# mpeg5/xeve

Measured on AMD Instinct MI355X. Metric: encoded frames/sec @ 2160p Baseline medium; SAD-kernel HBM GB/s vs peak, higher is better.
Workload: dtype s16 samples, s32/s64 accumulation, f64 cost comparisons (bit-exact)

## Files before the change

### xeve_amd/csrc/rdo.hip

```cpp
#include <cstdlib>
#include "xh_common.h"
#include "mc_cu.h"

extern "C" int xeve_hip_residual_rdoq_dev(const pel *org, int s_org, const pel *pred, int s_pred, const xeve_hip_job *jobs, int njobs, int log2w, int log2h,
                                          int bit_depth, int qp, int qscale, int dqscale, int is_intra_slice, double lambda, int ch_type, int tool_iqt,
                                          const xeve_hip_rdoq_est_full *est, const int32_t *est_idx, int16_t *coef, pel *rec, int s_rec, int32_t *nnz,
                                          int64_t *ssd, void *stream);

struct RdoK {
    int    n0, n1, ncomp, njobs, dir_unused;
    int    w, h, ws, hs, s_org_l, s_org_c;
    double lambda[3], wgt[2];
};

struct Cand {
    double cost_best;
    int    nnz_store[3], idx_best[3], cbf_idx[3], iy, iu, iv, tnnz, round4, win;
};

#define MAX_COST 1.7e+308

__device__ __forceinline__ void copy_state(xeve_hip_sbac *d, const xeve_hip_sbac *s)
{
    const unsigned *a = (const unsigned *)s;
// ... 208 lines not shown
}

__global__ void k_rdo_spec_decide(const xeve_hip_rdo_job *__restrict__ jobs, RdoK P, const long *ssd_y, const long *ssd_u, const long *ssd_v,
                                  const unsigned *__restrict__ bits, const unsigned *__restrict__ cbits, const xeve_hip_sbac *__restrict__ st_out,
                                  Cand *__restrict__ cand, xeve_hip_rdo_result *__restrict__ res, unsigned char *__restrict__ drop, xeve_hip_sbac *__restrict__ best)
{
    const int j = blockIdx.x * blockDim.x + threadIdx.x;
    if(j >= P.njobs) return;
    const xeve_hip_rdo_job J = jobs[j];
    Cand c = cand[j];
    long d0[3], d1[3];
    load_dist(ssd_y, ssd_u, ssd_v, j, P, d0, d1);
    const size_t N = P.njobs;
    auto wb = [&](int k) { return (double)(int)bits[(size_t)k * N + j]; };
    auto cb = [&](int lane, int which) { return (double)(int)cbits[4 * ((size_t)lane * N + j) + which]; };
    if(c.tnnz == 0) {
        c.cost_best = (double)d0[0] + (P.wgt[0] * (double)d0[1]) + (P.wgt[1] * (double)d0[2]);
        c.cost_best += wb(0) * P.lambda[0];
        c.win = 0;
        if(best) copy_state(best + j, st_out + j);
    }
    else {
        if(!J.dir_flag) {
            double cost = sum_cost(d0, d1, 0, 0, 0, P);
            cost += wb(0) * P.lambda[0];
            if(cost < c.cost_best) {
                c.cost_best = cost, c.cbf_idx[0] = c.cbf_idx[1] = c.cbf_idx[2] = 0, c.win = 0;
                if(best) copy_state(best + j, st_out + j);
            }
        }
        {
            double cost = sum_cost(d0, d1, c.iy, c.iu, c.iv, P);
            cost += wb(7) * P.lambda[0];
            if(cost < c.cost_best) {
                c.cost_best = cost, c.cbf_idx[0] = c.iy, c.cbf_idx[1] = c.iu, c.cbf_idx[2] = c.iv, c.win = 1;
                if(best) copy_state(best + j, st_out + 7 * N + j);
            }
        }
        int lane = 0;
        if(c.nnz_store[0] > 0) {
            double c0 = (double)d0[0] * 1.0, c1 = (double)d1[0] * 1.0;
            c0 += cb(0, 0) * P.lambda[0], c1 += cb(1, 0) * P.lambda[0];
            c.idx_best[0] = c1 < c0;
            lane |= c.idx_best[0];
        }
        if(c.nnz_store[1] > 0) {
            double c0 = (double)d0[1] * P.wgt[0], c1 = (double)d1[1] * P.wgt[0];
            c0 += cb(lane, 1) * P.lambda[1], c1 += cb(lane | 2, 1) * P.lambda[1];
            c.idx_best[1] = c1 < c0;
            lane |= c.idx_best[1] << 1;
        }
        if(c.nnz_store[2] > 0) {
            double c0 = (double)d0[2] * P.wgt[1], c1 = (double)d1[2] * P.wgt[1];
            c0 += cb(lane, 2) * P.lambda[2], c1 += cb(lane, 3) * P.lambda[2];
            c.idx_best[2] = c1 < c0;
        }
        int n[3] = {c.nnz_store[0], c.nnz_store[1], c.nnz_store[2]};
        if(c.idx_best[0] || c.idx_best[1] || c.idx_best[2]) {
            c.iy = c.idx_best[0], c.iu = c.idx_best[1], c.iv = c.idx_best[2];
            n[0] = c.iy ? n[0] : 0, n[1] = c.iu ? n[1] : 0, n[2] = c.iv ? n[2] : 0;
        }
        c.round4 = n[0] != c.nnz_store[0] || n[1] != c.nnz_store[1] || n[2] != c.nnz_store[2];
        if(c.round4) {
            const int k = (n[0] ? 1 : 0) | (n[1] ? 2 : 0) | (n[2] ? 4 : 0);
            double cost = sum_cost(d0, d1, c.iy, c.iu, c.iv, P);
            cost += wb(k) * P.lambda[0];
            if(cost < c.cost_best) {
                c.cost_best = cost, c.cbf_idx[0] = c.iy, c.cbf_idx[1] = c.iu, c.cbf_idx[2] = c.iv, c.win = 2;
                if(best) copy_state(best + j, st_out + (size_t)k * N + j);
            }
        }
    }
    cand[j] = c;
    xeve_hip_rdo_result r;
    r.cost = c.cost_best, r.pad_ = 0;
    for(int k = 0; k < 3; k++) {
        r.nnz[k] = c.tnnz != 0 && c.cbf_idx[k] ? c.nnz_store[k] : 0;
        drop[3 * j + k] = r.nnz[k] == 0 && c.nnz_store[k] != 0;
        r.dist[0][k] = d0[k], r.dist[1][k] = c.tnnz != 0 ? d1[k] : 0;
    }
    res[j] = r;
}

static int rdo_spec_limit()
{
    static const int v = getenv("XEVE_HIP_RDO_SPEC") ? atoi(getenv("XEVE_HIP_RDO_SPEC")) : 256;
    return v;
}
static bool rdo_use_spec(int njobs) { return njobs <= rdo_spec_limit(); }

static size_t al(size_t v) { return (v + 255) & ~(size_t)255; }

struct RdoLayout {
    size_t mc, rl, rc, est_idx, est, pred[3], rec[3], nnz[3], ssd[3], cand, prev, bj, bits, st_out, drop, mcws, bitws, total;
};
static RdoLayout rdo_layout(int njobs, int n0, int n1, int nstates, size_t rec_l, size_t rec_c, int w, int h, int nr0, int nr1)
{
    RdoLayout L;
    size_t o = 0, n = njobs;
    auto take = [&](size_t bytes) { size_t r = o; o += al(bytes); return r; };
    L.mc = take(n * sizeof(xeve_hip_cu_mc_job)), L.rl = take(n * sizeof(xeve_hip_job)), L.rc = take(n * sizeof(xeve_hip_job));
    L.est_idx = take(n * 4), L.est = take((size_t)nstates * sizeof(xeve_hip_rdoq_est_full));
    L.pred[0] = take(n * n0 * 2), L.pred[1] = take(n * n1 * 2 + 8), L.pred[2] = take(n * n1 * 2 + 8);
    (void)rec_l, (void)rec_c;
    L.rec[0] = take(n * n0 * 2), L.rec[1] = take(n * n1 * 2 + 8), L.rec[2] = take(n * n1 * 2 + 8);
    for(int k = 0; k < 3; k++) L.nnz[k] = take(n * 4), L.ssd[k] = take(n * 16);
    L.cand = take(n * sizeof(Cand)), L.prev = take(n * sizeof(xeve_hip_sbac));
    const size_t kinds = rdo_use_spec(njobs) ? 8 : 4;
    L.bj = take((kinds + 4) * n * sizeof(xeve_hip_cu_bits_job)), L.bits = take((kinds + 16) * n * 4), L.st_out = take(kinds * n * sizeof(xeve_hip_sbac));
    L.drop = take(3 * n);
    L.mcws = take(xeve_hip_mc_cu_workspace(njobs, w, h, nr0, nr1));
    L.bitws = take(xeve_hip_cu_bits_workspace((int)kinds * njobs, n * ((size_t)n0 + 2 * (size_t)n1)));
    L.total = o;
    return L;
}

extern "C" size_t xeve_hip_residue_rdo_workspace(int njobs, int nstates, const xeve_hip_rdo_params *p, int s_org_l, int s_org_c)
{
    if(!p || njobs <= 0) return 256;
    const int ws = p->chroma_format_idc <= 2, hs = p->chroma_format_idc <= 1;
    const int n0 = 1 << (p->log2_cuw + p->log2_cuh), n1 = p->chroma_format_idc ? n0 >> (ws + hs) : 0;
    return rdo_layout(njobs, n0, n1, nstates > 0 ? nstates : 1, (size_t)s_org_l * p->pic_h, (size_t)s_org_c * (p->pic_h >> hs), 1 << p->log2_cuw, 1 << p->log2_cuh,
                      p->num_refp[0], p->num_refp[1]).total;
}

static const int k_q_scale[6]  = {26214, 23302, 20560, 18396, 16384, 14764};
static const int k_dq_scale[6] = {40, 45, 51, 57, 64, 71};

extern "C" int xeve_hip_residue_rdo_jobs(const xeve_hip_pel *const org[3], int s_org_l, int s_org_c, const xeve_hip_refpic *refp, int s_l, int s_c,
                                         const xeve_hip_sbac *states, int nstates, const xeve_hip_rdo_params *p, const xeve_hip_rdo_job *jobs, int njobs,
                                         const int16_t (*coef_l)[8], const int16_t (*coef_c)[4], xeve_hip_rdo_result *results, int16_t *coef,
                                         xeve_hip_sbac *best, void *workspace, size_t workspace_bytes, void *stream)
{
    return xh_residue_rdo_jobs_x(org, s_org_l, s_org_c, refp, s_l, s_c, states, nstates, p, jobs, njobs, coef_l, coef_c, results, coef, best, workspace, workspace_bytes, stream,
                                 nullptr, 0);
}

int xh_residue_rdo_jobs_x(const xeve_hip_pel *const org[3], int s_org_l, int s_org_c, const xeve_hip_refpic *refp, int s_l, int s_c, const xeve_hip_sbac *states, int nstates,
                          const xeve_hip_rdo_params *p, const xeve_hip_rdo_job *jobs, int njobs, const int16_t (*coef_l)[8], const int16_t (*coef_c)[4],
                          xeve_hip_rdo_result *results, int16_t *coef, xeve_hip_sbac *best, void *workspace, size_t workspace_bytes, void *stream,
                          const void *est_shared, int keep_dropped)
{
    XH_ENTER();
    XH_REQUIRE(org && refp && states && nstates > 0 && p && jobs && njobs >= 0 && results && coef && workspace && coef_l);
    XH_REQUIRE(p->log2_cuw >= 2 && p->log2_cuw <= 6 && p->log2_cuh >= 2 && p->log2_cuh <= 6 && p->tool_iqt == 0);
    XH_REQUIRE(p->chroma_format_idc == 0 || p->chroma_format_idc == 1 || p->chroma_format_idc == 3);
    XH_REQUIRE(org[0] && (p->chroma_format_idc == 0 || (org[1] && org[2] && coef_c)));
    if(njobs == 0) return XEVE_HIP_OK;
    XH_REQUIRE(workspace_bytes >= xeve_hip_residue_rdo_workspace(njobs, nstates, p, s_org_l, s_org_c));
    const int idc = p->chroma_format_idc, ws = idc <= 2, hs = idc <= 1, bd = p->bit_depth;
    const int lw[3] = {p->log2_cuw, p->log2_cuw - ws, p->log2_cuw - ws}, lh[3] = {p->log2_cuh, p->log2_cuh - hs, p->log2_cuh - hs};
    RdoK P;
    P.n0 = 1 << (lw[0] + lh[0]), P.n1 = idc ? 1 << (lw[1] + lh[1]) : 0, P.ncomp = idc ? 3 : 1, P.njobs = njobs, P.dir_unused = 0;
    P.w = 1 << lw[0], P.h = 1 << lh[0], P.ws = ws, P.hs = hs, P.s_org_l = s_org_l, P.s_org_c = s_org_c;
    for(int k = 0; k < 3; k++) P.lambda[k] = p->lambda[k];
    P.wgt[0] = p->dist_chroma_weight[0], P.wgt[1] = p->dist_chroma_weight[1];
    const RdoLayout L = rdo_layout(njobs, P.n0, P.n1, nstates, (size_t)s_org_l * p->pic_h, (size_t)s_org_c * (p->pic_h >> hs), P.w, P.h, p->num_refp[0], p->num_refp[1]);
    char *W = (char *)workspace;
    auto *rl = (xeve_hip_job *)(W + L.rl), *rc = (xeve_hip_job *)(W + L.rc);
    int  *est_idx = (int *)(W + L.est_idx);
    auto *est = est_shared ? (xeve_hip_rdoq_est_full *)est_shared : (xeve_hip_rdoq_est_full *)(W + L.est);
    pel  *pred[3] = {(pel *)(W + L.pred[0]), (pel *)(W + L.pred[1]), (pel *)(W + L.pred[2])};
    pel  *rec[3]  = {(pel *)(W + L.rec[0]), (pel *)(W + L.rec[1]), (pel *)(W + L.rec[2])};
    int  *nnz[3]  = {(int *)(W + L.nnz[0]), (int *)(W + L.nnz[1]), (int *)(W + L.nnz[2])};
    long *ssd[3]  = {(long *)(W + L.ssd[0]), (long *)(W + L.ssd[1]), (long *)(W + L.ssd[2])};
    auto *cand = (Cand *)(W + L.cand);
    auto *prev = (xeve_hip_sbac *)(W + L.prev), *st_out = (xeve_hip_sbac *)(W + L.st_out);
    auto *bj = (xeve_hip_cu_bits_job *)(W + L.bj);
    auto *bits = (unsigned *)(W + L.bits);
    auto *drop = (unsigned char *)(W + L.drop);
    hipStream_t st = (hipStream_t)stream;
    const int   G  = (njobs + 255) / 256;
    int rc_;

    CuMcPrep C;
    rc_ = xh_mc_cu_prep_params(refp, p->num_refp[0], p->num_refp[1], p->pic_w, p->pic_h, njobs, P.w, P.h, idc, W + L.mcws, L.bitws - L.mcws, &C);
    if(rc_ != XEVE_HIP_OK) return rc_;
    k_rdo_prep<<<G, 256, 0, st>>>(jobs, P, C, rl, rc, est_idx);
    rc_ = xh_mc_cu_jobs_x(refp, p->num_refp[0], p->num_refp[1], s_l, s_c, p->pic_w, p->pic_h, nullptr, njobs, P.w, P.h, bd, bd, idc, coef_l, coef_c, pred[0],
                          pred[1], pred[2], W + L.mcws, L.bitws - L.mcws, stream, XH_MC_PREPPED);
    if(rc_ != XEVE_HIP_OK) return rc_;
    if(!est_shared) {
        rc_ = xeve_hip_rdoq_bit_est(states, nstates, est, stream);
        if(rc_ != XEVE_HIP_OK) return rc_;
    }
    int16_t *cf[3] = {coef, coef + (size_t)njobs * P.n0, coef + (size_t)njobs * (P.n0 + P.n1)};
    for(int k = 0; k < P.ncomp; k++) {
        const int q = p->qp[k];
        XH_REQUIRE(q >= 0 && q <= 51 + 6 * (bd - 8));
        rc_ = xeve_hip_residual_rdoq_dev(org[k], k ? s_org_c : s_org_l, pred[k], 1 << lw[k], k ? rc : rl, njobs, lw[k], lh[k], bd, q, k_q_scale[q % 6],
                                         k_dq_scale[q % 6] << (q / 6), p->slice_type == 2, p->lambda[k], k, p->tool_iqt, est, est_idx, cf[k], rec[k],
                                         -(1 << lw[k]), nnz[k], (int64_t *)ssd[k], stream);
        if(rc_ != XEVE_HIP_OK) return rc_;
    }
    xeve_hip_cu_bits_params bp;
    bp.log2_cuw = p->log2_cuw, bp.log2_cuh = p->log2_cuh, bp.slice_type = p->slice_type, bp.num_refp[0] = p->num_refp[0], bp.num_refp[1] = p->num_refp[1];
    bp.cm_init = 0, bp.chroma_format_idc = idc;
    const size_t coef_elems = (size_t)njobs * (P.n0 + 2 * (size_t)P.n1), bws = workspace_bytes - L.bitws;
    if(rdo_use_spec(njobs)) {
        xeve_hip_cu_bits_job *cj = bj + 8 * (size_t)njobs;
        unsigned             *cbits = bits + 8 * (size_t)njobs;
        k_rdo_spec_jobs<<<G, 256, 0, st>>>(jobs, P, nnz[0], nnz[1], nnz[2], cand, bj, cj);
        rc_ = xh_cu_bits_jobs_round(coef, coef_elems, states, bj, 8 * njobs, &bp, W + L.bitws, bws, bits, best ? st_out : nullptr, best != nullptr, 0, stream, 7 * njobs, njobs);
        if(rc_ != XEVE_HIP_OK) return rc_;
        rc_ = xh_cu_bits_chain_round(coef_elems, states, cj, 4 * njobs, &bp, W + L.bitws, bws, cbits, stream);
        if(rc_ != XEVE_HIP_OK) return rc_;
        k_rdo_spec_decide<<<G, 256, 0, st>>>(jobs, P, ssd[0], ssd[1], ssd[2], bits, cbits, st_out, cand, results, drop, best);
        if(!keep_dropped) k_rdo_zero_dropped<<<(3 * njobs + 3) / 4, 256, 0, st>>>(coef, drop, P);
        XH_HIP(hipGetLastError());
        return XEVE_HIP_OK;
    }
    k_rdo_round1<<<G, 256, 0, st>>>(jobs, P, nnz[0], nnz[1], nnz[2], cand, bj);
    rc_ = xh_cu_bits_jobs_round(coef, coef_elems, states, bj, 4 * njobs, &bp, W + L.bitws, bws, bits, st_out, best != nullptr, 0, stream, njobs, njobs);
    if(rc_ != XEVE_HIP_OK) return rc_;
    k_rdo_decide1<<<G, 256, 0, st>>>(jobs, P, ssd[0], ssd[1], ssd[2], bits, st_out, states, cand, prev, bj, best);
    if(P.ncomp > 1) {
        for(int comp = 1; comp <= 2; comp++) {
            rc_ = xh_cu_bits_jobs_round(coef, coef_elems, prev, bj, 2 * njobs, &bp, W + L.bitws, bws, bits, st_out, 0, 1, stream);
            if(rc_ != XEVE_HIP_OK) return rc_;
            k_rdo_decide_comp<<<G, 256, 0, st>>>(jobs, P, comp, ssd[0], ssd[1], ssd[2], bits, st_out, cand, prev, bj);
        }
    }
    else k_rdo_decide_comp<<<G, 256, 0, st>>>(jobs, P, 2, ssd[0], ssd[1], ssd[2], bits, st_out, cand, prev, bj);
    rc_ = xh_cu_bits_jobs_round(coef, coef_elems, states, bj, njobs, &bp, W + L.bitws, bws, bits, best ? st_out : nullptr, best != nullptr, 1, stream);
    if(rc_ != XEVE_HIP_OK) return rc_;
    k_rdo_finish<<<G, 256, 0, st>>>(jobs, P, ssd[0], ssd[1], ssd[2], bits, cand, results, drop, st_out, best);
    if(!keep_dropped) k_rdo_zero_dropped<<<(3 * njobs + 3) / 4, 256, 0, st>>>(coef, drop, P);
    XH_HIP(hipGetLastError());
    return XEVE_HIP_OK;
}

struct SkipK {
    int    njobs, S, mc, isb, n0, n1, ncomp, ws, hs, s_org_l, s_org_c, best_shift;
    double lambda0, wgt[2];
};

__global__ void k_skip_prep(const xeve_hip_skip_job *__restrict__ jobs, SkipK P, CuMcPrep C, xeve_hip_cu_mc_job *__restrict__ mc, xeve_hip_job *__restrict__ rl,
                            xeve_hip_job *__restrict__ rc, xeve_hip_cu_bits_job *__restrict__ bj, unsigned char *__restrict__ valid, int *__restrict__ zero)
{
    const int t = blockIdx.x * blockDim.x + threadIdx.x;
    if(t < 64) zero[t] = 0;
    if(t >= P.njobs * P.S) return;
    const int j = t / P.S, s = t % P.S;
    const int i0 = P.isb ? s / P.mc : s, i1 = P.isb ? s % P.mc : 0;
    const xeve_hip_skip_job J = jobs[j];
    const int cnt1 = P.isb ? J.ncand : 1;
    bool ok = i0 < J.ncand && i1 < cnt1;
    for(int k = 0; k < 3; k++) {
        if(k < i0 && J.mvp[0][k][0] == J.mvp[0][i0][0] && J.mvp[0][k][1] == J.mvp[0][i0][1]) ok = false;
        if(k < i1 && J.mvp[1][k][0] == J.mvp[1][i1][0] && J.mvp[1][k][1] == J.mvp[1][i1][1]) ok = false;
    }
    xeve_hip_cu_mc_job m;
    m.x = J.x, m.y = J.y, m.mv[0][0] = J.mvp[0][i0][0], m.mv[0][1] = J.mvp[0][i0][1], m.mv[1][0] = J.mvp[1][i1][0], m.mv[1][1] = J.mvp[1][i1][1];
    m.refi[0] = J.refi_pred[0][i0], m.refi[1] = P.isb ? J.refi_pred[1][i1] : -1, m.pad_[0] = m.pad_[1] = 0;
    if(m.refi[0] < 0 && m.refi[1] < 0) ok = false;
    if(!ok) m.refi[0] = m.refi[1] = -1;
    mc[t] = m;
    xh_cu_mc_prep_one(m, t, C);
    rl[t] = xh_make_job(J.y, P.s_org_l, J.x, t * P.n0);
    rc[t] = xh_make_job(J.y >> P.hs, P.s_org_c, J.x >> P.ws, t * P.n1);
    xeve_hip_cu_bits_job b;
    b.coef_off[0] = b.coef_off[1] = b.coef_off[2] = 0, b.nnz[0] = b.nnz[1] = b.nnz[2] = 0, b.sbac = J.sbac;
    b.mvd[0][0] = b.mvd[0][1] = b.mvd[1][0] = b.mvd[1][1] = 0, b.refi[0] = b.refi[1] = 0;
    b.mvp_idx[0] = (uint8_t)i0, b.mvp_idx[1] = (uint8_t)i1, b.mode = XEVE_HIP_BITS_CU_SKIP, b.dir_flag = 0, b.ctx_skip = J.ctx_skip, b.ctx_pred_mode = 0;
    bj[t] = b;
    valid[t] = ok;
}

__global__ void k_skip_decide_copy(const xeve_hip_skip_job *__restrict__ jobs, SkipK P, const xeve_hip_cu_mc_job *__restrict__ mc, const unsigned char *__restrict__ valid,
                                   const long *__restrict__ ssd_y, const long *__restrict__ ssd_u, const long *__restrict__ ssd_v, const unsigned *__restrict__ bits,
                                   xeve_hip_skip_result *__restrict__ res, int *__restrict__ win, const pel *__restrict__ sy, const pel *__restrict__ su,
                                   const pel *__restrict__ sv, pel *__restrict__ py, pel *__restrict__ pu, pel *__restrict__ pv, const xeve_hip_sbac *__restrict__ st,
                                   xeve_hip_sbac *__restrict__ best)
{
    __shared__ int s_win;
    const int j = blockIdx.x;
    if(threadIdx.x == 0) {
        double cost_best = MAX_COST;
        int    sb = -1;
        long   ssd_best = 1L << P.best_shift;
        for(int s = 0; s < P.S; s++) {
            const int t = j * P.S + s;
            if(!valid[t]) continue;
            const long cy = ssd_y[t], cu = P.ncomp > 1 ? ssd_u[t] : 0, cv = P.ncomp > 1 ? ssd_v[t] : 0;
            double cost = (double)cy + (P.wgt[0] * (double)cu) + (P.wgt[1] * (double)cv);
            cost += (double)(int)bits[t] * P.lambda0;
            if(cost < cost_best) cost_best = cost, sb = s, ssd_best = cy + cu + cv;
        }
// ... 120 lines not shown
```

### xeve_amd/csrc/sbac.hip

```cpp
#include <cstdlib>
#include <cstring>
#include <type_traits>
#include "xh_common.h"

#define NCTX XEVE_HIP_SBAC_NCTX
#define QCAP 48

struct CuBitsK {
    int n[3], log2n[3];
    int slice_type, num_refp[2], cm_init, idc;
    const uint16_t *scan[3];
};

__device__ __forceinline__ unsigned ev_pack(int v, int run, int at_end)
{
    const unsigned a = (unsigned)(v < 0 ? -v : v) & 0xFFFFu;
    return ((a - 1) & 0x7FFFu) | ((unsigned)(v < 0) << 15) | ((unsigned)run << 16) | ((unsigned)at_end << 28);
}

__device__ __forceinline__ unsigned coded_mask(const xeve_hip_cu_bits_job &j)
{
    if(j.mode == XEVE_HIP_BITS_CU_SKIP || j.mode == XEVE_HIP_BITS_MVP || j.mode == XEVE_HIP_BITS_INTRA_DIR) return 0;
    unsigned m = (j.nnz[0] ? 1u : 0u) | (j.nnz[1] ? 2u : 0u) | (j.nnz[2] ? 4u : 0u);
    if(j.mode == XEVE_HIP_BITS_ECO_COEF) return m & ((j.dir_flag >> 2) & 7u);
// ... 398 lines not shown
            }
            if(FULL) sb_drain(s);
        }
        cur = nxt, rem -= 16;
    }
}

template <bool FULL>
__device__ __forceinline__ void code_events(Sbac &s, CtxTab s_ctx, int lane, const unsigned *__restrict__ ev, int nevents, int num_sig, int ch, int cm_init)
{
    auto bin = [&](int ci, unsigned b) {
        const unsigned m = sb_encode<FULL>(s, s_ctx[ci][lane], b, false);
        s_ctx[ci][lane] = (uint16_t)m;
        if(FULL) sb_drain(s);
    };
    unsigned plev = 5;
    for(int e = 0; e < nevents; e++) {
        const unsigned cur = ev[e], run = (cur >> 16) & 0xFFF, lev1 = cur & 0x7FFF, sign = (cur >> 15) & 1, at_end = (cur >> 28) & 1;
        const int t0 = cm_init == 1 ? (int)(plev << 1) + ch * 12 : ch * 2;
        bin(XEVE_HIP_CTX_RUN + t0, run != 0);
        if(run) {
            for(unsigned i = 1; i < run; i++) bin(XEVE_HIP_CTX_RUN + t0 + 1, 1);
            bin(XEVE_HIP_CTX_RUN + t0 + 1, 0);
        }
        bin(XEVE_HIP_CTX_LEVEL + t0, lev1 != 0);
        if(lev1) {
            for(unsigned i = 1; i < lev1; i++) bin(XEVE_HIP_CTX_LEVEL + t0 + 1, 1);
            bin(XEVE_HIP_CTX_LEVEL + t0 + 1, 0);
        }
        (void)sb_encode<FULL>(s, 0, sign, true);
        if(FULL) sb_drain(s);
        num_sig--;
        if(!at_end) bin(XEVE_HIP_CTX_LAST + ch, num_sig == 0);
        plev = lev1 < 5 ? lev1 : 5u;
    }
}

template <bool FULL>
__device__ __forceinline__ void code_block(Sbac &s, CtxTab s_ctx, int lane, const unsigned char *__restrict__ bins, const unsigned *__restrict__ ev, int coef_off, int nnz,
                                           int c, int cm_init, unsigned long long *slow)
{
    const unsigned *hdr = reinterpret_cast<const unsigned *>(bins + (size_t)coef_off * BINK);
    const unsigned nb = hdr[0], nev = hdr[1];
    if(nb != BIN_OVF && nev == (unsigned)nnz) code_string<FULL>(s, s_ctx, lane, reinterpret_cast<const unsigned char *>(hdr) + BIN_HDR, (int)nb);
    else {
        if(slow) atomicAdd(XH_PROF_SLOT(slow), 1ull);
        code_events<FULL>(s, s_ctx, lane, ev + coef_off, (int)(nev < (unsigned)nnz ? nev : (unsigned)nnz), nnz, c != 0, cm_init);
    }
}

__device__ __forceinline__ void sbac_load(Sbac &s, const xeve_hip_sbac &in, CtxTab s_ctx, int lane, bool continue_coder, const uint32_t *s_tab)
{
    s.tab = s_tab;
    s.range = in.range, s.shifts = s.bins = 0;
    s.code = in.code & 0x7FFFF, s.fifo = 0, s.cnt = 0, s.cb = 11, s.sff = s.sz = s.pb = s.ipb = s.bc = 0;
    if(continue_coder) {
        s.code = in.code, s.cb = in.code_bits, s.sff = in.stacked_ff, s.sz = in.stacked_zero, s.pb = in.pending_byte, s.ipb = in.is_pending_byte;
        s.bc = in.bitcounter, s.bins = in.bin_counter;
    }
    for(int i = 0; i < NCTX; i++) s_ctx[i][lane] = in.ctx[i];
    s_ctx[BYP][lane] = 0;
}

__device__ unsigned long long g_bins_hist[16 * 32];
extern "C" int xeve_hip_prof_cu_bits_hist(unsigned long long *out, int reset)
{
    XH_ENTER();
    unsigned long long h[16 * 32];
    XH_HIP(hipDeviceSynchronize());
    XH_HIP(hipMemcpyFromSymbol(h, HIP_SYMBOL(g_bins_hist), sizeof(h)));
    if(out)
        for(int b = 0; b < 32; b++) {
            out[b] = 0;
            for(int s = 0; s < 16; s++) out[b] += h[s * 32 + b];
        }
    if(reset) {
        memset(h, 0, sizeof(h));
        XH_HIP(hipMemcpyToSymbol(HIP_SYMBOL(g_bins_hist), h, sizeof(h)));
    }
    return XEVE_HIP_OK;
}

template <bool FULL>
__global__ __launch_bounds__(64) void k_cu_bits(const xeve_hip_sbac *__restrict__ sin, const xeve_hip_cu_bits_job *__restrict__ jobs, int njobs, CuBitsK P,
                                                const unsigned char *__restrict__ bins, const unsigned *__restrict__ ev, unsigned *__restrict__ bits,
                                                xeve_hip_sbac *__restrict__ sout, unsigned long long *__restrict__ units, unsigned long long *__restrict__ slow)
{
    __shared__ uint16_t s_ctx[NCTX + 1][64];
    __shared__ uint8_t  s_q[QCAP][64];
    __shared__ uint32_t s_tab[1024];
    load_model_tab(s_tab);
    const int lane = threadIdx.x, j = blockIdx.x * 64 + lane;
    if(j >= njobs) return;
    const xeve_hip_cu_bits_job J = jobs[j];
    const xeve_hip_sbac &in = sin[J.sbac];
    const bool cont = FULL && J.mode == XEVE_HIP_BITS_ECO_COEF && (J.dir_flag & XEVE_HIP_ECO_NO_RESET);
    Sbac s;
    sbac_load(s, in, s_ctx, lane, cont, s_tab);
    Queue Q{&s_q[0][lane], 0, 0};
    const unsigned coded = q_header(Q, J, P);
    code_queue<FULL>(s, s_ctx, s_q, lane, Q.n < QCAP ? Q.n : QCAP);
    for(int base = QCAP; base < Q.n; base += QCAP) {
        Queue W{&s_q[0][lane], 0, base};
        (void)q_header(W, J, P);
        code_queue<FULL>(s, s_ctx, s_q, lane, Q.n - base < QCAP ? Q.n - base : QCAP);
    }
    for(int c = 0; c < 3; c++)
        if((coded >> c) & 1) code_block<FULL>(s, s_ctx, lane, bins, ev, J.coef_off[c], J.nnz[c], c, P.cm_init, slow);
    bits[j] = s.shifts;
    if(units) {
        const unsigned nb = s.bins - (cont ? in.bin_counter : 0u);
        atomicAdd(&g_bins_hist[((blockIdx.x & 15) << 5) + (nb ? 32 - __clz(nb) : 0)], 1ull);
    }
    if(units) {
        unsigned *cnt = reinterpret_cast<unsigned *>(&s_q[0][0]);
        const bool first = lane == (int)(__ffsll((long long)__ballot(true)) - 1);
        if(first) *cnt = 0;
        atomicAdd(cnt, s.bins - (cont ? in.bin_counter : 0u));
        if(first) atomicAdd(XH_PROF_SLOT(units), (unsigned long long)*cnt);
    }
    if(!FULL && sout) {
        xeve_hip_sbac &o = sout[j];
        o.range = s.range, o.code = 0, o.code_bits = 11, o.stacked_ff = o.stacked_zero = o.pending_byte = o.is_pending_byte = o.bitcounter = 0;
        o.bin_counter = s.bins;
        for(int i = 0; i < NCTX; i++) o.ctx[i] = s_ctx[i][lane];
    }
    if(FULL) {
        sb_drain(s);
        bits[j] = s.bc + 8 * (s.sz + s.sff) + 8 * (s.ipb ? 1 : 0) + 8 - s.cb + 3;
        xeve_hip_sbac &o = sout[j];
        o.range = s.range, o.code = s.code, o.code_bits = s.cb, o.stacked_ff = s.sff, o.stacked_zero = s.sz;
        o.pending_byte = s.pb, o.is_pending_byte = s.ipb, o.bitcounter = s.bc, o.bin_counter = s.bins;
        for(int i = 0; i < NCTX; i++) o.ctx[i] = s_ctx[i][lane];
    }
}

__global__ __launch_bounds__(64) void k_cu_bits_chain(const xeve_hip_sbac *__restrict__ sin, const xeve_hip_cu_bits_job *__restrict__ jobs, int njobs, CuBitsK P,
                                                      const unsigned char *__restrict__ bins, const unsigned *__restrict__ ev, unsigned *__restrict__ out,
                                                      unsigned long long *__restrict__ units, unsigned long long *__restrict__ slow)
{
    __shared__ uint16_t s_ctx[NCTX + 1][64];
    __shared__ uint8_t  s_q[QCAP][64];
    __shared__ uint32_t s_tab[1024];
    load_model_tab(s_tab);
    const int lane = threadIdx.x, j = blockIdx.x * 64 + lane;
    if(j >= njobs) return;
    const xeve_hip_cu_bits_job J = jobs[j];
    if(J.mode == XEVE_HIP_BITS_CU_SKIP) return;
    Sbac s;
    sbac_load(s, sin[J.sbac], s_ctx, lane, false, s_tab);
    const int keep[3] = {J.dir_flag & 1, (J.dir_flag >> 1) & 1, 1};
    unsigned total_bins = 0;
    for(int c = 0; c < 3; c++) {
        if(J.nnz[c] <= 0) continue;
        xeve_hip_cu_bits_job T = J;
        T.mode = (uint8_t)(XEVE_HIP_BITS_COMP_Y + c);
        if(c == 2) {
            T.nnz[2] = 0;
            Queue Q0{&s_q[0][lane], 0, 0};
            (void)q_header(Q0, T, P);
            Sbac t = s;
            for(int i = 0; i < Q0.n; i++) {
                const unsigned e = s_q[i][lane];
                (void)sb_encode<false>(t, s_ctx[e >> 1][lane], e & 1, (e >> 1) == BYP);
            }
            out[4 * j + 2] = t.shifts;
            T.nnz[2] = J.nnz[2];
        }
        else if(!keep[c]) T.nnz[c] = 0;
        Queue Q{&s_q[0][lane], 0, 0};
        const unsigned coded = q_header(Q, T, P);
        code_queue<false>(s, s_ctx, s_q, lane, Q.n);
        if((coded >> c) & 1) code_block<false>(s, s_ctx, lane, bins, ev, J.coef_off[c], J.nnz[c], c, P.cm_init, slow);
        out[4 * j + (c == 2 ? 3 : c)] = s.shifts;
        total_bins += s.bins;
        s.shifts = 0, s.bins = 0;
    }
    if(units) {
        unsigned *cnt = reinterpret_cast<unsigned *>(&s_q[0][0]);
        const bool first = lane == (int)(__ffsll((long long)__ballot(true)) - 1);
        if(first) *cnt = 0;
        atomicAdd(cnt, total_bins);
        if(first) atomicAdd(XH_PROF_SLOT(units), (unsigned long long)*cnt);
    }
}

static size_t ws_bins_off(size_t coef_elems) { return (sizeof(unsigned) * coef_elems + 255) & ~(size_t)255; }
static size_t ws_nev_off(size_t coef_elems) { return ws_bins_off(coef_elems) + (((size_t)BINK * coef_elems + 64 + 255) & ~(size_t)255); }
extern "C" size_t xeve_hip_cu_bits_workspace(int njobs, size_t coef_elems)
{
    const size_t n = njobs > 0 ? njobs : 0;
    return ws_nev_off(coef_elems) + ((sizeof(int) * 3 * n + 255) & ~(size_t)255) + n + 256;
}

static int cu_bits_launch(const int16_t *coef, size_t coef_elems, const xeve_hip_sbac *sbac_in, const xeve_hip_cu_bits_job *jobs, int njobs,
                          const xeve_hip_cu_bits_params *p, void *workspace, size_t workspace_bytes, uint32_t *bits, xeve_hip_sbac *sbac_out, bool full,
                          void *stream, bool reuse_events = false, int ev_first = 0, int ev_count = -1);

extern "C" int xeve_hip_cu_bits_jobs(const int16_t *coef, size_t coef_elems, const xeve_hip_sbac *sbac_in, const xeve_hip_cu_bits_job *jobs, int njobs,
                                     const xeve_hip_cu_bits_params *p, void *workspace, size_t workspace_bytes, uint32_t *bits,
                                     xeve_hip_sbac *sbac_out, void *stream)
{
    return cu_bits_launch(coef, coef_elems, sbac_in, jobs, njobs, p, workspace, workspace_bytes, bits, sbac_out, sbac_out != nullptr, stream);
}

extern "C" int xeve_hip_cu_bits_jobs_chain(const int16_t *coef, size_t coef_elems, const xeve_hip_sbac *sbac_in, const xeve_hip_cu_bits_job *jobs, int njobs,
                                           const xeve_hip_cu_bits_params *p, void *workspace, size_t workspace_bytes, uint32_t *bits,
                                           xeve_hip_sbac *state_out, void *stream)
{
    return cu_bits_launch(coef, coef_elems, sbac_in, jobs, njobs, p, workspace, workspace_bytes, bits, state_out, false, stream);
}

int xh_cu_bits_jobs_round(const int16_t *coef, size_t coef_elems, const xeve_hip_sbac *sbac_in, const xeve_hip_cu_bits_job *jobs, int njobs,
                          const xeve_hip_cu_bits_params *p, void *workspace, size_t workspace_bytes, uint32_t *bits, xeve_hip_sbac *state_out, int full, int reuse,
                          void *stream, int ev_first, int ev_count)
{
    return cu_bits_launch(coef, coef_elems, sbac_in, jobs, njobs, p, workspace, workspace_bytes, bits, state_out, full != 0, stream, reuse != 0, ev_first, ev_count);
}

static int fill_k(CuBitsK &P, const xeve_hip_cu_bits_params *p)
{
    const int ws = p->chroma_format_idc <= 2, hs = p->chroma_format_idc <= 1;
    for(int c = 0; c < 3; c++) {
        const int lw = p->log2_cuw - (c ? ws : 0), lh = p->log2_cuh - (c ? hs : 0);
        P.log2n[c] = lw + lh, P.n[c] = 1 << (lw + lh);
        const int rc = xh_get_scan(lw, lh, &P.scan[c]);
        if(rc != XEVE_HIP_OK) return rc;
    }
    P.slice_type = p->slice_type, P.num_refp[0] = p->num_refp[0], P.num_refp[1] = p->num_refp[1];
    P.cm_init = p->cm_init, P.idc = p->chroma_format_idc;
    return XEVE_HIP_OK;
}

int xh_cu_bits_chain_round(size_t coef_elems, const xeve_hip_sbac *sbac_in, const xeve_hip_cu_bits_job *jobs, int njobs, const xeve_hip_cu_bits_params *p,
                           void *workspace, size_t workspace_bytes, uint32_t *out, void *stream)
{
    XH_ENTER();
    XH_REQUIRE(p && njobs >= 0 && sbac_in && jobs && out && workspace && workspace_bytes >= xeve_hip_cu_bits_workspace(njobs, coef_elems));
    if(njobs == 0) return XEVE_HIP_OK;
    CuBitsK P;
    const int rc = fill_k(P, p);
    if(rc != XEVE_HIP_OK) return rc;
    char *W = (char *)workspace;
    hipStream_t st = (hipStream_t)stream;
    XhProf prof(XH_PROF_CU_BITS, st);
    k_cu_bits_chain<<<(njobs + 63) / 64, 64, 0, st>>>(sbac_in, jobs, njobs, P, (const unsigned char *)(W + ws_bins_off(coef_elems)), (const unsigned *)W, out,
                                                     xh_prof_units(XH_PROF_CU_BITS), xh_prof_units(XH_PROF_CU_BITS_SLOW));
    XH_HIP(hipGetLastError());
    return XEVE_HIP_OK;
}

static int cu_bits_launch(const int16_t *coef, size_t coef_elems, const xeve_hip_sbac *sbac_in, const xeve_hip_cu_bits_job *jobs, int njobs,
                          const xeve_hip_cu_bits_params *p, void *workspace, size_t workspace_bytes, uint32_t *bits, xeve_hip_sbac *sbac_out, bool full,
                          void *stream, bool reuse_events, int ev_first, int ev_count)
{
    XH_ENTER();
    XH_REQUIRE(p && njobs >= 0);
    XH_REQUIRE(p->log2_cuw >= 2 && p->log2_cuw <= 6 && p->log2_cuh >= 2 && p->log2_cuh <= 6);
    XH_REQUIRE(p->slice_type >= 0 && p->slice_type <= 2 && p->chroma_format_idc >= 0 && p->chroma_format_idc <= 3);
    XH_REQUIRE(p->num_refp[0] >= 0 && p->num_refp[0] <= 21 && p->num_refp[1] >= 0 && p->num_refp[1] <= 21);
    if(njobs == 0) return XEVE_HIP_OK;
    if(xh_count_states()) full = false;
    XH_REQUIRE(sbac_in && jobs && bits && workspace);
    XH_REQUIRE(workspace_bytes >= xeve_hip_cu_bits_workspace(njobs, coef_elems));
    CuBitsK P;
    {
        const int rc = fill_k(P, p);
        if(rc != XEVE_HIP_OK) return rc;
    }
    char          *W    = (char *)workspace;
    unsigned      *ev   = (unsigned *)W;
    unsigned char *bins = (unsigned char *)(W + ws_bins_off(coef_elems));
    int           *nev  = (int *)(W + ws_nev_off(coef_elems));
    XH_REQUIRE(((uintptr_t)workspace & 15) == 0);
    hipStream_t st = (hipStream_t)stream;
    if(ev_count < 0) ev_first = 0, ev_count = njobs;
    XH_REQUIRE(ev_first >= 0 && ev_first + ev_count <= njobs);
    const long items = 3L * ev_count;
    if(!coef || reuse_events || ev_count == 0) {}
    else if(P.n[0] <= 64) {
        const long waves = (items + 3) / 4;
        k_coef_events<16><<<(unsigned)((waves + 3) / 4), 256, 0, st>>>(coef, jobs + ev_first, ev_count, P, ev, nev, bins);
    }
    else k_coef_events<64><<<(unsigned)((items + 3) / 4), 256, 0, st>>>(coef, jobs + ev_first, ev_count, P, ev, nev, bins);
    {
        XhProf prof(XH_PROF_CU_BITS, st);
        unsigned long long *units = xh_prof_units(XH_PROF_CU_BITS), *slow = xh_prof_units(XH_PROF_CU_BITS_SLOW);
        if(full) k_cu_bits<true><<<(njobs + 63) / 64, 64, 0, st>>>(sbac_in, jobs, njobs, P, bins, ev, bits, sbac_out, units, slow);
        else k_cu_bits<false><<<(njobs + 63) / 64, 64, 0, st>>>(sbac_in, jobs, njobs, P, bins, ev, bits, sbac_out, units, slow);
    }
    XH_HIP(hipGetLastError());
    return XEVE_HIP_OK;
}


extern "C" int xeve_hip_eco_coef_host(xeve_hip_sbac *state, const int16_t *coef_y, const int16_t *coef_u, const int16_t *coef_v, int log2_cuw, int log2_cuh,
                                      const int32_t nnz[3], int flags, int chroma_format_idc, int cm_init)
{
    XH_ENTER();
    XH_REQUIRE(state && coef_y && nnz && log2_cuw >= 2 && log2_cuw <= 6 && log2_cuh >= 2 && log2_cuh <= 6 && chroma_format_idc >= 0 && chroma_format_idc <= 3);
    XH_REQUIRE(chroma_format_idc == 0 || (coef_u && coef_v));
    const int ws = chroma_format_idc <= 2, hs = chroma_format_idc <= 1;
    const size_t n0 = (size_t)1 << (log2_cuw + log2_cuh), n1 = chroma_format_idc ? n0 >> (ws + hs) : 0, ne = n0 + 2 * n1;
    xeve_hip_cu_bits_params p;
    p.log2_cuw = log2_cuw, p.log2_cuh = log2_cuh, p.slice_type = 0, p.num_refp[0] = p.num_refp[1] = 0, p.cm_init = cm_init, p.chroma_format_idc = chroma_format_idc;
    xeve_hip_cu_bits_job j;
    memset(&j, 0, sizeof(j));
    j.coef_off[0] = 0, j.coef_off[1] = (int)n0, j.coef_off[2] = (int)(n0 + n1), j.nnz[0] = nnz[0], j.nnz[1] = nnz[1], j.nnz[2] = nnz[2];
    j.mode = XEVE_HIP_BITS_ECO_COEF, j.dir_flag = (uint8_t)(flags | XEVE_HIP_ECO_NO_RESET);
    const size_t o_job = (ne * 2 + 255) & ~(size_t)255, o_st = o_job + 256, o_bits = o_st + 2 * 256, o_ws = o_bits + 256;
    const size_t wsb = xeve_hip_cu_bits_workspace(1, ne);
    char *d = nullptr;
    XH_HIP(hipMalloc((void **)&d, o_ws + wsb));
    int rc = XEVE_HIP_OK;
    auto up = [&](size_t off, const void *src, size_t bytes) { if(rc == XEVE_HIP_OK && hipMemcpy(d + off, src, bytes, hipMemcpyHostToDevice) != hipSuccess) rc = XEVE_HIP_ERR_DEVICE; };
    up(0, coef_y, n0 * 2);
    if(n1) up(n0 * 2, coef_u, n1 * 2), up((n0 + n1) * 2, coef_v, n1 * 2);
    up(o_job, &j, sizeof(j)), up(o_st, state, sizeof(*state));
    if(rc == XEVE_HIP_OK)
        rc = xeve_hip_cu_bits_jobs((const int16_t *)d, ne, (const xeve_hip_sbac *)(d + o_st), (const xeve_hip_cu_bits_job *)(d + o_job), 1, &p, d + o_ws, wsb,
                                   (uint32_t *)(d + o_bits), (xeve_hip_sbac *)(d + o_st + 256), nullptr);
    else xh_set_error("xeve_hip_eco_coef_host: staging failed");
    if(rc == XEVE_HIP_OK && hipMemcpy(state, d + o_st + 256, sizeof(*state), hipMemcpyDeviceToHost) != hipSuccess) {
        xh_set_error("xeve_hip_eco_coef_host: copy back failed");
        rc = XEVE_HIP_ERR_DEVICE;
    }
    (void)hipFree(d);
    return rc;
}
```

### xeve_amd/csrc/xh_common.h

```cpp
#pragma once
#include <hip/hip_runtime.h>
#include <stdint.h>
#include "../../include/xeve_hip.h"

typedef int16_t pel;

#define XH_WAVE 64

void xh_set_error(const char *fmt, ...);
bool xh_ready();

#define XH_HIP(expr)                                                                               \
    do {                                                                                           \
        hipError_t e_ = (expr);                                                                    \
        if(e_ != hipSuccess) {                                                                     \
            xh_set_error("%s failed: %s (%s:%d)", #expr, hipGetErrorString(e_), __FILE__, __LINE__); \
            return XEVE_HIP_ERR_DEVICE;                                                            \
        }                                                                                          \
    } while(0)

#define XH_REQUIRE(cond)                                                         \
    do {                                                                         \
        if(!(cond)) {                                                            \
            xh_set_error("invalid argument: %s (%s:%d)", #cond, __FILE__, __LINE__); \
            return XEVE_HIP_ERR_ARG;                                             \
        }                                                                        \
    } while(0)

#define XH_ENTER()                                                   \
    do {                                                             \
        if(!xh_ready()) {                                            \
            xh_set_error("xeve_hip_init() has not been called");     \
            return XEVE_HIP_ERR_UNINIT;                              \
        }                                                            \
    } while(0)

enum { XH_PROF_SEARCH = 0, XH_PROF_SPEL = 1, XH_PROF_CU_BITS = 2, XH_PROF_MC = 3, XH_PROF_RESID = 4, XH_PROF_RDOQ = 5, XH_PROF_CU_BITS_SLOW = 6, XH_PROF_WALK = 7 };
bool  xh_prof_on(int cls);
void *xh_prof_begin(int cls, hipStream_t st);
void  xh_prof_end(void *tok, hipStream_t st);
#define XH_PROF_STRIPES 256
unsigned long long *xh_prof_units(int cls);
#define XH_PROF_SLOT(units) ((units) + (blockIdx.x & (XH_PROF_STRIPES - 1)))
void *xh_prof_begin_kernel(int cls, hipEvent_t *start, hipEvent_t *stop);
void  xh_prof_end_kernel(void *tok);
struct XhProf {
    void       *tok;
    hipStream_t st;
    XhProf(int cls, hipStream_t s) : tok(xh_prof_on(cls) ? xh_prof_begin(cls, s) : nullptr), st(s) {}
    ~XhProf() { if(tok) xh_prof_end(tok, st); }
};

bool     xh_resident_on();
void    *xh_resident(const void *host, size_t bytes);
void     xh_resident_free_all();
uint32_t xh_generation();

struct RdoParams {
    int  shift_fwd, shift_inv;
    int  q_scale, q_shift, q_offset;
    long z_scale, z_thr;
    long dq_scale;
    int  dq_shift, dq_offset;
    int  ssd_shift, maxv;
    int  stage;
};

int xh_get_scan(int log2w, int log2h, const uint16_t **out);
const int *xh_entropy_table();
int xh_cu_bits_jobs_round(const int16_t *coef, size_t coef_elems, const xeve_hip_sbac *sbac_in, const xeve_hip_cu_bits_job *jobs, int njobs,
                          const xeve_hip_cu_bits_params *p, void *workspace, size_t workspace_bytes, uint32_t *bits, xeve_hip_sbac *state_out, int full, int reuse,
                          void *stream, int ev_first = 0, int ev_count = -1);
int xh_cu_bits_chain_round(size_t coef_elems, const xeve_hip_sbac *sbac_in, const xeve_hip_cu_bits_job *jobs, int njobs, const xeve_hip_cu_bits_params *p,
                           void *workspace, size_t workspace_bytes, uint32_t *out, void *stream);
#define XH_MAX_PLANES 16
struct XhSearchPlanes {
    const pel *ref[XH_MAX_PLANES];
    int        refi_bits[XH_MAX_PLANES], range[XH_MAX_PLANES], refi[XH_MAX_PLANES];
    int        n, per_plane;
    const unsigned char *job_plane;
    int        vh;
};

int xh_vh();
struct XhVhScope {
    int prev;
    explicit XhVhScope(int vh);
    ~XhVhScope();
};
int xh_count_states();
void xh_walk_load(long chains);
struct XhCountStatesScope {
    int prev;
    XhCountStatesScope();
    ~XhCountStatesScope();
};
__host__ __device__ __forceinline__ int xh_vh_base(int y, int vh) { return vh > 0 ? (y / vh) * vh : 0; }
#define XH_OFF2_HALF 0x40000000
#define XH_FRAC_HALF 0x100
inline bool xh_walk_only(const xeve_hip_tree_params *p) { return p->rdo_dbk != 0 || (p->ip.slice_type != 2 && p->min_cu < 8); }

struct XhJob {
    size_t off1;
    int    off2;
};
__host__ __device__ __forceinline__ XhJob xh_job(const xeve_hip_job &j)
{
    const bool half = ((uint32_t)j.off2 & 0xC0000000u) == (uint32_t)XH_OFF2_HALF;
    XhJob r;
    r.off1 = half ? (size_t)(uint32_t)j.off1 << 1 : (size_t)(uint32_t)j.off1, r.off2 = half ? (int)((uint32_t)j.off2 & 0x3FFFFFFFu) : j.off2;
    return r;
}
__host__ __device__ __forceinline__ size_t xh_u(size_t off) { return off; }
__host__ __device__ __forceinline__ size_t xh_u(int off) { return (size_t)(uint32_t)off; }
__host__ __device__ __forceinline__ xeve_hip_job xh_make_job(size_t o, int off2)
{
    xeve_hip_job j;
    if((o & 1) || off2 < 0 || off2 >= XH_OFF2_HALF) j.off1 = (int)(uint32_t)o, j.off2 = off2;
    else j.off1 = (int)(uint32_t)(o >> 1), j.off2 = off2 | XH_OFF2_HALF;
    return j;
}
__host__ __device__ __forceinline__ xeve_hip_job xh_make_job(long y, long stride, long x, int off2) { return xh_make_job((size_t)(y * stride + x), off2); }
__device__ __forceinline__ int xh_plane_of_job(const unsigned char *job_plane, int per_plane, int j) { return job_plane ? job_plane[j] : j / per_plane; }
struct XhInterCand {
    const uint32_t *map_scu;
    const uint8_t  *map_tidx;
    const int16_t  *map_mv, *col0, *col1;
    int             w_scu, scuw, scuh, isb, vh;
};
int xh_pinter_analyze_cu_jobs_x(const xeve_hip_pel *const org[3], int s_org_l, int s_org_c, const xeve_hip_refpic *refp, int s_l, int s_c, const xeve_hip_sbac *states,
                                int nstates, const xeve_hip_inter_params *p, xeve_hip_inter_job *jobs, int njobs, const int16_t (*coef_l)[8], const int16_t (*coef_c)[4],
                                xeve_hip_inter_result *results, int16_t *coef, xeve_hip_pel *rec_y, xeve_hip_pel *rec_u, xeve_hip_pel *rec_v, xeve_hip_pel *pred_y,
                                xeve_hip_sbac *next_best, void *workspace, size_t workspace_bytes, void *stream, const XhInterCand *cand, const void *est_shared);
int xh_pintra_analyze_cu_jobs_x(const xeve_hip_pel *const org[3], int s_org_l, int s_org_c, const xeve_hip_pel *const mod[3], int s_mod_l, int s_mod_c, const uint32_t *map_scu,
                                const int8_t *map_ipm, const uint8_t *map_tidx, const int64_t *pic_elems, const xeve_hip_sbac *states, int nstates,
                                const xeve_hip_intra_params *p, const xeve_hip_intra_job *jobs, int njobs, xeve_hip_intra_result *results, int16_t *coef, xeve_hip_pel *rec,
                                xeve_hip_sbac *best, void *workspace, size_t workspace_bytes, void *stream, const void *est_shared);
int xh_residue_rdo_jobs_x(const xeve_hip_pel *const org[3], int s_org_l, int s_org_c, const xeve_hip_refpic *refp, int s_l, int s_c, const xeve_hip_sbac *states, int nstates,
                          const xeve_hip_rdo_params *p, const xeve_hip_rdo_job *jobs, int njobs, const int16_t (*coef_l)[8], const int16_t (*coef_c)[4],
                          xeve_hip_rdo_result *results, int16_t *coef, xeve_hip_sbac *best, void *workspace, size_t workspace_bytes, void *stream,
                          const void *est_shared, int keep_dropped);
int xh_residual_back(const pel *org, int s_org, const pel *pred, int s_pred, const xeve_hip_job *jobs, int njobs, int log2w, int log2h, int bit_depth, int qp, int dqscale,
                     const int16_t *coef, pel *rec, int s_rec, int32_t *nnz, int64_t *ssd, hipStream_t st);
struct EpzsState {
    uint32_t cost;
    int16_t  mv[2];
    int32_t  tmpstep, searches;
    int32_t  mot_bits;
};
struct XhSpelFinish {
    const EpzsState    *state;
    xeve_hip_me_result *out;
};
int xh_me_spel_pattern_jobs_x(const pel *org0, int s_org, const pel *org_bi, const pel *ref0, int s_ref, const xeve_hip_spel_job *jobs, int njobs, int log2w,
                              int log2h, int bit_depth, const int16_t (*coef)[8], const xeve_hip_spel_params *params, const int32_t *extra,
                              xeve_hip_me_result *results, void *workspace, size_t workspace_bytes, void *stream, const XhSearchPlanes *planes = nullptr, const struct XhSpelFinish *finish = nullptr);
int xh_me_epzs_jobs_planes(const pel *org0, int s_org, const pel *org_bi, const pel *ref0, int s_ref, const xeve_hip_epzs_job *jobs, int njobs, int log2w, int log2h,
// ... 101 lines not shown
```

Before: 18.73.

## Fuse speculative cu-bits and chain rounds into one kernel launch

```diff
diff --git a/xeve_amd/csrc/rdo.hip b/xeve_amd/csrc/rdo.hip
--- a/xeve_amd/csrc/rdo.hip
+++ b/xeve_amd/csrc/rdo.hip
@@ -314,12 +314,18 @@
     res[j] = r;
 }
 
+#define RDO_SPEC_LOG2_DEFAULT 0
 static int rdo_spec_limit()
 {
     static const int v = getenv("XEVE_HIP_RDO_SPEC") ? atoi(getenv("XEVE_HIP_RDO_SPEC")) : 256;
     return v;
 }
-static bool rdo_use_spec(int njobs) { return njobs <= rdo_spec_limit(); }
+static int rdo_spec_log2()
+{
+    static const int v = getenv("XEVE_HIP_RDO_SPEC_LOG2") ? atoi(getenv("XEVE_HIP_RDO_SPEC_LOG2")) : RDO_SPEC_LOG2_DEFAULT;
+    return v;
+}
+static bool rdo_use_spec(int njobs, int n0) { return rdo_spec_limit() > 0 && (njobs <= rdo_spec_limit() || n0 <= (1 << rdo_spec_log2())); }
 
 static size_t al(size_t v) { return (v + 255) & ~(size_t)255; }
 
@@ -338,7 +344,7 @@
     L.rec[0] = take(n * n0 * 2), L.rec[1] = take(n * n1 * 2 + 8), L.rec[2] = take(n * n1 * 2 + 8);
     for(int k = 0; k < 3; k++) L.nnz[k] = take(n * 4), L.ssd[k] = take(n * 16);
     L.cand = take(n * sizeof(Cand)), L.prev = take(n * sizeof(xeve_hip_sbac));
-    const size_t kinds = rdo_use_spec(njobs) ? 8 : 4;
+    const size_t kinds = rdo_use_spec(njobs, n0) ? 8 : 4;
     L.bj = take((kinds + 4) * n * sizeof(xeve_hip_cu_bits_job)), L.bits = take((kinds + 16) * n * 4), L.st_out = take(kinds * n * sizeof(xeve_hip_sbac));
     L.drop = take(3 * n);
     L.mcws = take(xeve_hip_mc_cu_workspace(njobs, w, h, nr0, nr1));
@@ -429,13 +435,12 @@
     bp.log2_cuw = p->log2_cuw, bp.log2_cuh = p->log2_cuh, bp.slice_type = p->slice_type, bp.num_refp[0] = p->num_refp[0], bp.num_refp[1] = p->num_refp[1];
     bp.cm_init = 0, bp.chroma_format_idc = idc;
     const size_t coef_elems = (size_t)njobs * (P.n0 + 2 * (size_t)P.n1), bws = workspace_bytes - L.bitws;
-    if(rdo_use_spec(njobs)) {
+    if(rdo_use_spec(njobs, P.n0)) {
         xeve_hip_cu_bits_job *cj = bj + 8 * (size_t)njobs;
         unsigned             *cbits = bits + 8 * (size_t)njobs;
         k_rdo_spec_jobs<<<G, 256, 0, st>>>(jobs, P, nnz[0], nnz[1], nnz[2], cand, bj, cj);
-        rc_ = xh_cu_bits_jobs_round(coef, coef_elems, states, bj, 8 * njobs, &bp, W + L.bitws, bws, bits, best ? st_out : nullptr, best != nullptr, 0, stream, 7 * njobs, njobs);
-        if(rc_ != XEVE_HIP_OK) return rc_;
-        rc_ = xh_cu_bits_chain_round(coef_elems, states, cj, 4 * njobs, &bp, W + L.bitws, bws, cbits, stream);
+        rc_ = xh_cu_bits_spec_round(coef, coef_elems, states, bj, 8 * njobs, cj, 4 * njobs, &bp, W + L.bitws, bws, bits, best ? st_out : nullptr, best != nullptr, cbits, stream,
+                                    7 * njobs, njobs);
         if(rc_ != XEVE_HIP_OK) return rc_;
         k_rdo_spec_decide<<<G, 256, 0, st>>>(jobs, P, ssd[0], ssd[1], ssd[2], bits, cbits, st_out, cand, results, drop, best);
         if(!keep_dropped) k_rdo_zero_dropped<<<(3 * njobs + 3) / 4, 256, 0, st>>>(coef, drop, P);
diff --git a/xeve_amd/csrc/sbac.hip b/xeve_amd/csrc/sbac.hip
--- a/xeve_amd/csrc/sbac.hip
+++ b/xeve_amd/csrc/sbac.hip
@@ -504,15 +504,12 @@
 }
 
 template <bool FULL>
-__global__ __launch_bounds__(64) void k_cu_bits(const xeve_hip_sbac *__restrict__ sin, const xeve_hip_cu_bits_job *__restrict__ jobs, int njobs, CuBitsK P,
-                                                const unsigned char *__restrict__ bins, const unsigned *__restrict__ ev, unsigned *__restrict__ bits,
-                                                xeve_hip_sbac *__restrict__ sout, unsigned long long *__restrict__ units, unsigned long long *__restrict__ slow)
-{
-    __shared__ uint16_t s_ctx[NCTX + 1][64];
-    __shared__ uint8_t  s_q[QCAP][64];
-    __shared__ uint32_t s_tab[1024];
-    load_model_tab(s_tab);
-    const int lane = threadIdx.x, j = blockIdx.x * 64 + lane;
+__device__ __forceinline__ void cu_bits_body(CtxTab s_ctx, uint8_t (*s_q)[64], const uint32_t *s_tab, int wg, const xeve_hip_sbac *__restrict__ sin,
+                                             const xeve_hip_cu_bits_job *__restrict__ jobs, int njobs, const CuBitsK &P, const unsigned char *__restrict__ bins,
+                                             const unsigned *__restrict__ ev, unsigned *__restrict__ bits, xeve_hip_sbac *__restrict__ sout,
+                                             unsigned long long *__restrict__ units, unsigned long long *__restrict__ slow)
+{
+    const int lane = threadIdx.x, j = wg * 64 + lane;
     if(j >= njobs) return;
     const xeve_hip_cu_bits_job J = jobs[j];
     const xeve_hip_sbac &in = sin[J.sbac];
@@ -557,15 +554,24 @@
     }
 }
 
-__global__ __launch_bounds__(64) void k_cu_bits_chain(const xeve_hip_sbac *__restrict__ sin, const xeve_hip_cu_bits_job *__restrict__ jobs, int njobs, CuBitsK P,
-                                                      const unsigned char *__restrict__ bins, const unsigned *__restrict__ ev, unsigned *__restrict__ out,
-                                                      unsigned long long *__restrict__ units, unsigned long long *__restrict__ slow)
+template <bool FULL>
+__global__ __launch_bounds__(64) void k_cu_bits(const xeve_hip_sbac *__restrict__ sin, const xeve_hip_cu_bits_job *__restrict__ jobs, int njobs, CuBitsK P,
+                                                const unsigned char *__restrict__ bins, const unsigned *__restrict__ ev, unsigned *__restrict__ bits,
+                                                xeve_hip_sbac *__restrict__ sout, unsigned long long *__restrict__ units, unsigned long long *__restrict__ slow)
 {
     __shared__ uint16_t s_ctx[NCTX + 1][64];
     __shared__ uint8_t  s_q[QCAP][64];
     __shared__ uint32_t s_tab[1024];
     load_model_tab(s_tab);
-    const int lane = threadIdx.x, j = blockIdx.x * 64 + lane;
+    cu_bits_body<FULL>(s_ctx, s_q, s_tab, blockIdx.x, sin, jobs, njobs, P, bins, ev, bits, sout, units, slow);
+}
+
+__device__ __forceinline__ void cu_bits_chain_body(CtxTab s_ctx, uint8_t (*s_q)[64], const uint32_t *s_tab, int wg, const xeve_hip_sbac *__restrict__ sin,
+                                                   const xeve_hip_cu_bits_job *__restrict__ jobs, int njobs, const CuBitsK &P, const unsigned char *__restrict__ bins,
+                                                   const unsigned *__restrict__ ev, unsigned *__restrict__ out, unsigned long long *__restrict__ units,
+                                                   unsigned long long *__restrict__ slow)
+{
+    const int lane = threadIdx.x, j = wg * 64 + lane;
     if(j >= njobs) return;
     const xeve_hip_cu_bits_job J = jobs[j];
     if(J.mode == XEVE_HIP_BITS_CU_SKIP) return;
@@ -607,6 +613,31 @@
     }
 }
 
+__global__ __launch_bounds__(64) void k_cu_bits_chain(const xeve_hip_sbac *__restrict__ sin, const xeve_hip_cu_bits_job *__restrict__ jobs, int njobs, CuBitsK P,
+                                                      const unsigned char *__restrict__ bins, const unsigned *__restrict__ ev, unsigned *__restrict__ out,
+                                                      unsigned long long *__restrict__ units, unsigned long long *__restrict__ slow)
+{
+    __shared__ uint16_t s_ctx[NCTX + 1][64];
+    __shared__ uint8_t  s_q[QCAP][64];
+    __shared__ uint32_t s_tab[1024];
+    load_model_tab(s_tab);
+    cu_bits_chain_body(s_ctx, s_q, s_tab, blockIdx.x, sin, jobs, njobs, P, bins, ev, out, units, slow);
+}
+
+__global__ __launch_bounds__(64) void k_cu_bits_spec(const xeve_hip_sbac *__restrict__ sin, const xeve_hip_cu_bits_job *__restrict__ jobs, int njobs,
+                                                     const xeve_hip_cu_bits_job *__restrict__ cjobs, int ncjobs, CuBitsK P, const unsigned char *__restrict__ bins,
+                                                     const unsigned *__restrict__ ev, unsigned *__restrict__ bits, xeve_hip_sbac *__restrict__ sout,
+                                                     unsigned *__restrict__ cbits, unsigned long long *__restrict__ units, unsigned long long *__restrict__ slow)
+{
+    __shared__ uint16_t s_ctx[NCTX + 1][64];
+    __shared__ uint8_t  s_q[QCAP][64];
+    __shared__ uint32_t s_tab[1024];
+    load_model_tab(s_tab);
+    const int nwg = (njobs + 63) / 64;
+    if((int)blockIdx.x < nwg) cu_bits_body<false>(s_ctx, s_q, s_tab, blockIdx.x, sin, jobs, njobs, P, bins, ev, bits, sout, units, slow);
+    else cu_bits_chain_body(s_ctx, s_q, s_tab, (int)blockIdx.x - nwg, sin, cjobs, ncjobs, P, bins, ev, cbits, units, slow);
+}
+
 static size_t ws_bins_off(size_t coef_elems) { return (sizeof(unsigned) * coef_elems + 255) & ~(size_t)255; }
 static size_t ws_nev_off(size_t coef_elems) { return ws_bins_off(coef_elems) + (((size_t)BINK * coef_elems + 64 + 255) & ~(size_t)255); }
 extern "C" size_t xeve_hip_cu_bits_workspace(int njobs, size_t coef_elems)
@@ -617,7 +648,8 @@
 
 static int cu_bits_launch(const int16_t *coef, size_t coef_elems, const xeve_hip_sbac *sbac_in, const xeve_hip_cu_bits_job *jobs, int njobs,
                           const xeve_hip_cu_bits_params *p, void *workspace, size_t workspace_bytes, uint32_t *bits, xeve_hip_sbac *sbac_out, bool full,
-                          void *stream, bool reuse_events = false, int ev_first = 0, int ev_count = -1);
+                          void *stream, bool reuse_events = false, int ev_first = 0, int ev_count = -1, const xeve_hip_cu_bits_job *cjobs = nullptr, int ncjobs = 0,
+                          uint32_t *cbits = nullptr);
 
 extern "C" int xeve_hip_cu_bits_jobs(const int16_t *coef, size_t coef_elems, const xeve_hip_sbac *sbac_in, const xeve_hip_cu_bits_job *jobs, int njobs,
                                      const xeve_hip_cu_bits_params *p, void *workspace, size_t workspace_bytes, uint32_t *bits,
@@ -672,9 +704,22 @@
     return XEVE_HIP_OK;
 }
 
+int xh_cu_bits_spec_round(const int16_t *coef, size_t coef_elems, const xeve_hip_sbac *sbac_in, const xeve_hip_cu_bits_job *jobs, int njobs,
+                          const xeve_hip_cu_bits_job *cjobs, int ncjobs, const xeve_hip_cu_bits_params *p, void *workspace, size_t workspace_bytes, uint32_t *bits,
+                          xeve_hip_sbac *state_out, int full, uint32_t *cbits, void *stream, int ev_first, int ev_count)
+{
+    XH_REQUIRE(cjobs && cbits && ncjobs >= 0 && ncjobs <= njobs);
+    if((full && !xh_count_states()) || ncjobs == 0) {
+        const int rc = cu_bits_launch(coef, coef_elems, sbac_in, jobs, njobs, p, workspace, workspace_bytes, bits, state_out, full != 0, stream, false, ev_first, ev_count);
+        if(rc != XEVE_HIP_OK) return rc;
+        return xh_cu_bits_chain_round(coef_elems, sbac_in, cjobs, ncjobs, p, workspace, workspace_bytes, cbits, stream);
+    }
+    return cu_bits_launch(coef, coef_elems, sbac_in, jobs, njobs, p, workspace, workspace_bytes, bits, state_out, false, stream, false, ev_first, ev_count, cjobs, ncjobs, cbits);
+}
+
 static int cu_bits_launch(const int16_t *coef, size_t coef_elems, const xeve_hip_sbac *sbac_in, const xeve_hip_cu_bits_job *jobs, int njobs,
                           const xeve_hip_cu_bits_params *p, void *workspace, size_t workspace_bytes, uint32_t *bits, xeve_hip_sbac *sbac_out, bool full,
-                          void *stream, bool reuse_events, int ev_first, int ev_count)
+                          void *stream, bool reuse_events, int ev_first, int ev_count, const xeve_hip_cu_bits_job *cjobs, int ncjobs, uint32_t *cbits)
 {
     XH_ENTER();
     XH_REQUIRE(p && njobs >= 0);
@@ -709,6 +754,8 @@
         XhProf prof(XH_PROF_CU_BITS, st);
         unsigned long long *units = xh_prof_units(XH_PROF_CU_BITS), *slow = xh_prof_units(XH_PROF_CU_BITS_SLOW);
         if(full) k_cu_bits<true><<<(njobs + 63) / 64, 64, 0, st>>>(sbac_in, jobs, njobs, P, bins, ev, bits, sbac_out, units, slow);
+        else if(ncjobs > 0)
+            k_cu_bits_spec<<<(njobs + 63) / 64 + (ncjobs + 63) / 64, 64, 0, st>>>(sbac_in, jobs, njobs, cjobs, ncjobs, P, bins, ev, bits, sbac_out, cbits, units, slow);
         else k_cu_bits<false><<<(njobs + 63) / 64, 64, 0, st>>>(sbac_in, jobs, njobs, P, bins, ev, bits, sbac_out, units, slow);
     }
     XH_HIP(hipGetLastError());
diff --git a/xeve_amd/csrc/xh_common.h b/xeve_amd/csrc/xh_common.h
--- a/xeve_amd/csrc/xh_common.h
+++ b/xeve_amd/csrc/xh_common.h
@@ -73,6 +73,9 @@
                           void *stream, int ev_first = 0, int ev_count = -1);
 int xh_cu_bits_chain_round(size_t coef_elems, const xeve_hip_sbac *sbac_in, const xeve_hip_cu_bits_job *jobs, int njobs, const xeve_hip_cu_bits_params *p,
                            void *workspace, size_t workspace_bytes, uint32_t *out, void *stream);
+int xh_cu_bits_spec_round(const int16_t *coef, size_t coef_elems, const xeve_hip_sbac *sbac_in, const xeve_hip_cu_bits_job *jobs, int njobs,
+                          const xeve_hip_cu_bits_job *cjobs, int ncjobs, const xeve_hip_cu_bits_params *p, void *workspace, size_t workspace_bytes, uint32_t *bits,
+                          xeve_hip_sbac *state_out, int full, uint32_t *cbits, void *stream, int ev_first, int ev_count);
 #define XH_MAX_PLANES 16
 struct XhSearchPlanes {
     const pel *ref[XH_MAX_PLANES];
```

Result: no change. 18.71, median of 2 (-0.1%).
